# TUI-NICR/EMSANet

Measured on AMD Instinct MI355X. Metric: images/sec (640x480 RGB-D, bs=32/GPU) fwd+bwd, higher is better.
Workload: dtype f32; 1 GPU; BASELINE.json configs[1]: full EMSANet RGB-D (resnet34-NBt1D x2, SE-add fusion, PPM, semantic+instance+orientation+scene heads), 640x480, bs=32/GPU, f32, train mode (BN batch stats, Dropout2d), step = fwd + bwd (fixed output cotangents) + grad all-reduce + SGD-nesterov update at lr 0 (fixed weights) replayed from a hipGraph; global_batch=32, parallelism=dp1, weights=random init (deterministic), mode=train-hipgraph

## Files before the change

### emsanet_amd/_lib.py

```python
import ctypes
import os
from ctypes import POINTER, Structure, c_char_p, c_float, c_int, c_int8, c_int32, c_int64, c_uint32, c_void_p

LIB_PATH = os.environ.get('EMSA_LIB') or os.path.join(
    os.path.dirname(os.path.abspath(__file__)), 'lib', 'libemsanet_hip.so')


class EmsaPackJob(Structure):
    _fields_ = [('src', c_void_p), ('dst0', c_void_p), ('dst1', c_void_p), ('cout', c_int32),
                ('cin', c_int32), ('kh', c_int32), ('kw', c_int32), ('kind', c_int32),
                ('first_block', c_int32), ('cout_total', c_int32), ('cout_off', c_int32),
                ('cin_total', c_int32), ('cin_off', c_int32)]


PACK_GEMM = 0
PACK_WINO = 1
PACK_GEMM_16 = {1: 2, 2: 3}
PACK_COPY = 4
PACK_FRAG_16 = {1: 5, 2: 6}
PACK_WINO2D = 7


class EmsaDropoutJob(Structure):
    _fields_ = [('offset', c_int64), ('c', c_int32), ('layer_id', c_uint32), ('p', c_float),
# ... 14 lines not shown
        ('out_pix_img', c_int32), ('out_pix_row', c_int32), ('out_pix_px', c_int32),
        ('out_pix_off', c_int32),
    ]


class EmsaTargetScale(Structure):
    _fields_ = [('scale', c_int32), ('sigma', c_int32), ('semantic', c_void_p), ('center', c_void_p),
                ('offset', c_void_p), ('foreground', c_void_p), ('orientation', c_void_p),
                ('orientation_foreground', c_void_p)]


class EmsaExportJob(Structure):
    _fields_ = [('src0', c_void_p), ('src1', c_void_p), ('depth', c_void_p), ('lut', c_void_p),
                ('dst', c_void_p), ('divisor', c_int64), ('max_depth', ctypes.c_double),
                ('kind', c_int32), ('src0_dtype', c_int32), ('src1_dtype', c_int32),
                ('depth_dtype', c_int32), ('lut_size', c_int32), ('add', c_int32), ('h', c_int32),
                ('w', c_int32)]


class EmsaNormalScale(Structure):
    _fields_ = [('scale', c_int32), ('reserved', c_int32), ('out', c_void_p)]


_P = c_void_p
_GP = POINTER(EmsaConvGeom)
_TP = POINTER(EmsaTargetScale)

SIGNATURES = {
    'emsa_arch': (c_char_p, []),
    'emsa_version': (c_int, []),
    'emsa_set_batch_invariant': (c_int, [c_int]),
    'emsa_conv_igemm': (c_int, [_GP, _P, _P, _P, _P, _P, _P, _P, _P, c_int32, _P, c_int32, c_int32, _P]),
    'emsa_conv_stats_rows': (c_int, [_GP]),
    'emsa_conv1d_wino_supported': (c_int, [_GP]),
    'emsa_conv1d_wino_stats_rows': (c_int, [_GP]),
    'emsa_conv_relu_bits_words': (c_int64, [c_int64, c_int32]),
    'emsa_conv1d_wino_bnb': (c_int, [_GP, _P, _P, _P, _P, c_int32, _P, c_int32, _P, _P, _P, _P, _P,
                                     c_int32, _P]),
    'emsa_conv_igemm_bnb_t': (c_int, [c_int32, _GP, _P, _P, _P, _P, c_int32, _P, c_int32, _P, _P, _P, _P,
                                      _P, c_int32, _P]),
    'emsa_bn_bwd_apply_rows_t': (c_int, [c_int32, _P, _P, _P, _P, _P, _P, c_int32, c_int32, c_int64,
                                         c_int32, c_int32, _P, _P, _P, _P]),
    'emsa_conv1d_wino': (c_int, [_GP, _P, _P, _P, _P, _P, _P, _P, _P, c_int32, _P, c_int32, c_int32, _P,
                                 _P, _P]),
    'emsa_memset_async': (c_int, [_P, c_int32, c_int64, _P]),
    'emsa_graph_count_nodes': (c_int, [_P, POINTER(c_int32), POINTER(c_int32), POINTER(c_int32)]),
    'emsa_graph_replace_memsets': (c_int, [_P, POINTER(c_int32)]),
    'emsa_dropout2d_mask_batch': (c_int, [_P, _P, c_int32, c_int32, c_int32, c_uint32, _P, _P]),
    'emsa_to_nhwc_t': (c_int, [c_int32, _P, _P, c_int32, c_int32, c_int32, c_int32, c_int64, c_int64,
                               c_int64, c_int64, _P]),
    'emsa_conv1d_wino_set_spec': (c_int, [c_int32]),
    'emsa_wino_set_u_tiled': (c_int, [c_int32]),
    'emsa_conv1d_wino_spec_launches': (c_int, []),
    'emsa_conv1d_wino_resmask_supported': (c_int, [_GP, c_int32]),
    'emsa_conv1d_wino_resmask': (c_int, [_GP, _P, _P, _P, _P, c_int32, _P, _P]),
    'emsa_bn_act_fwd_wbits': (c_int, [_P, _P, _P, _P, _P, _P, c_int32, c_int64, c_int32, c_int32, _P, _P]),
    'emsa_bn_act_fwd_raff': (c_int, [_P] * 8 + [c_int32, c_int64, c_int32, c_int32, _P, c_int32, _P]),
    'emsa_bn_bwd_reduce_wbits': (c_int, [_P, _P, _P, _P, _P, _P, c_int32, c_int64, c_int32, _P, _P]),
    'emsa_bn_bwd_apply_wbits': (c_int, [_P] * 8 + [c_int32, c_int32, c_int64, c_int32, c_int32] + [_P] * 5),
    'emsa_conv1d_wino_inbn': (c_int, [_GP, _P, _P, _P, _P, _P, _P, _P, c_int32, _P, _P]),
    'emsa_conv_wgrad_inbn': (c_int, [_GP, _P, _P, _P, _P, _P, _P, _P, _P]),
    'emsa_conv_wgrad_inbn_t': (c_int, [c_int32, _GP, _P, _P, _P, _P, _P, _P, _P, _P]),
    'emsa_conv_wgrad_multi_inbn_t': (c_int, [c_int32, c_int32, _GP, POINTER(c_void_p), POINTER(c_void_p),
                                             POINTER(c_void_p), POINTER(c_void_p), _P,
                                             POINTER(c_void_p), POINTER(c_void_p), _P]),
    'emsa_conv1d_rs_inbn_t': (c_int, [c_int32, _GP, _P, _P, _P, _P, _P, _P, _P, c_int32, _P]),
    'emsa_bn_bwd_reduce_aff_t': (c_int, [c_int32, _P, _P, _P, _P, _P, _P, c_int32, c_int64, c_int32, _P, _P]),
    'emsa_bn_bwd_apply_aff_t': (c_int, [c_int32, _P, _P, _P, _P, _P, _P, _P, _P, c_int32, c_int32, c_int64,
                                        c_int32, _P, _P, _P, _P]),
    'emsa_conv_wgrad_multi_ws_bytes': (c_int64, [c_int32, c_int32, _GP]),
    'emsa_conv_wgrad_multi_t': (c_int, [c_int32, c_int32, _GP, POINTER(c_void_p), POINTER(c_void_p),
                                        POINTER(c_void_p), POINTER(c_void_p), _P, _P]),
    'emsa_pack_wino': (c_int, [_P, _P, _P, c_int32, c_int32, c_int32, _P]),
    'emsa_pack_batch': (c_int, [_P, c_int32, c_int32, _P]),
    'emsa_conv_wino2d_supported': (c_int, [_GP]),
    'emsa_conv_wino2d_stats_rows': (c_int, [_GP]),
    'emsa_conv_wino2d': (c_int, [_GP, _P, _P, _P, _P, _P, _P, _P, _P, c_int32, _P, c_int32, c_int32, _P]),
    'emsa_conv_wgrad_wino2d_supported': (c_int, [c_int32, _GP]),
    'emsa_conv_wgrad_wino2d_ws_bytes': (c_int64, [c_int32, _GP]),
    'emsa_conv_wgrad_wino2d_split_steps': (c_int, [c_int32, _GP]),
    'emsa_conv_wgrad_wino2d': (c_int, [c_int32, _GP, _P, _P, _P, _P, _P, c_int32, _P]),
    'emsa_pack_wino2d': (c_int, [_P, _P, _P, c_int32, c_int32, _P]),
    'emsa_pack_wino2d_packed': (c_int, [_P, _P, c_int32, c_int32, c_int32, _P]),
    'emsa_pack_wino_packed': (c_int, [_P, _P, c_int32, c_int32, c_int32, c_int32, _P]),
    'emsa_conv_wgrad_ws_bytes': (c_int64, [_GP]),
    'emsa_conv_wgrad': (c_int, [_GP, _P, _P, _P, _P, _P, _P]),
    'emsa_pack_weight_fwd': (c_int, [_P, _P] + [c_int32] * 8 + [_P]),
    'emsa_pack_weight_dgrad': (c_int, [_P, _P] + [c_int32] * 8 + [_P]),
    'emsa_unpack_wgrad': (c_int, [_P, _P] + [c_int32] * 8 + [_P]),
    'emsa_pack_weight_pair': (c_int, [_P, _P, _P] + [c_int32] * 4 + [_P]),
    'emsa_stem_pack_input': (c_int, [_P, _P, c_int32, c_int32, c_int32, c_int32, _P]),
    'emsa_stem_pack_weight': (c_int, [_P, _P, c_int32, c_int32, _P]),
    'emsa_stem_pack_input_rows_t': (c_int, [c_int32, _P, _P, c_int32, c_int32, c_int32, _P]),
    'emsa_stem_pack_weight_rows_t': (c_int, [c_int32, _P, _P, c_int32, _P]),
    'emsa_stem_unpack_wgrad_rows': (c_int, [_P, _P, c_int32, _P]),
    'emsa_stem_unpack_wgrad': (c_int, [_P, _P, c_int32, c_int32, _P]),
    'emsa_bn_finalize': (c_int, [_P, c_int32, c_int32, c_int64, _P, _P, c_float, c_float,
                                 _P, _P, _P, _P, _P, _P, _P, _P]),
    'emsa_bn_finalize_ws_bytes': (c_int, [c_int32]),
    'emsa_bn_fold': (c_int, [_P, _P, _P, _P, c_float, c_int32, _P, _P, _P, _P]),
    'emsa_relu_mask_words': (c_int64, [c_int64]),
    'emsa_bn_act_fwd': (c_int, [_P, _P, _P, _P, _P, _P, c_int32, c_int64, c_int32, c_int32, _P,
                                _P]),
    'emsa_bn_bwd_reduce': (c_int, [_P, _P, _P, _P, _P, _P, _P, c_int32, c_int64, c_int32, c_int32,
                                   _P, _P]),
    'emsa_bn_bwd_rows': (c_int, [c_int64, c_int32]),
# ... 215 lines not shown
```

### emsanet_amd/csrc/conv_wino.hip

```cpp
#include <atomic>
#include <cstdlib>
#include <type_traits>

#include "common.h"
#include "prof.h"

namespace {

constexpr int kWK = 16;
constexpr int kWLD = kWK;
constexpr int kPairs = 32;

typedef unsigned int u32x4w __attribute__((ext_vector_type(4)));
typedef __bf16 wbf16x8 __attribute__((ext_vector_type(8)));
constexpr uint32_t kOOBw = 0x80000000u;
__device__ __forceinline__ __amdgpu_buffer_rsrc_t wrsrc(const void* p, uint32_t bytes) {
  return __builtin_amdgcn_make_buffer_rsrc(const_cast<void*>(p), 0, (int)bytes, 0x00020000);
}
__device__ __forceinline__ float4 wbuf_ld4(__amdgpu_buffer_rsrc_t r, uint32_t off) {
  return __builtin_bit_cast(float4, __builtin_amdgcn_raw_buffer_load_b128(r, (int)off, 0, 0));
}
__device__ __forceinline__ float4 wbuf_ld4s(__amdgpu_buffer_rsrc_t r, uint32_t voff, uint32_t soff) {
  return __builtin_bit_cast(float4,
                            __builtin_amdgcn_raw_buffer_load_b128(r, (int)voff, (int)soff, 0));
}
typedef float wf32x2 __attribute__((ext_vector_type(2)));
typedef unsigned int wu32x2 __attribute__((ext_vector_type(2)));

struct WinoArgs {
  const float* in;
  const float* u;
  float* out;
  const float* bias;
  float* stats;
  const float* scale;
  const float* shift;
  const float* residual;
  const float* mask_src;
  const uint64_t* mask_bits;
  int mask_res;
  uint64_t* relu_bits;
  const float* bnb_mean;
  const float* bnb_invstd;
  float* bnb_out;
  int bnb_rows_alloc;
  const float* in_scale;
  const float* in_shift;
  int ld_out, ld_res, ld_mask, act;
  int L, PL, A, MP;
  int k_ch, n_ch;
  int R, c_in, ksteps_c;
  int u_tiled;
  int in_simg, in_sa, in_sb;
  int px_simg, px_sa, px_sb;
  int tiles_m, tiles_n, ksteps;
  uint32_t in_bytes, u_bytes;
  uint32_t mul_pl, sh_pl, mul_a, sh_a;
};

__device__ __forceinline__ int wswz(int row, int c4) {
  return row * kWLD + (c4 ^ (((row >> 2) & 3) << 2));
}

__device__ __forceinline__ uint32_t wdiv(uint32_t n, uint32_t mul, uint32_t sh) {
  return (__umulhi(n, mul) + n) >> sh;
}

#ifndef EMSA_WINO_ST_AUX
#define EMSA_WINO_ST_AUX 0
#endif
#ifndef EMSA_WINO_PRIO
#define EMSA_WINO_PRIO 2
#endif
enum : int {
  kOBias = 1, kORelu = 2, kORBits = 4, kOStats = 8, kOMBits = 16, kORes = 32, kOMRes = 64
};
template <int kWN, bool BF16 = false, bool BNB = false, bool INBN = false, int OPT = -1>
__global__ __launch_bounds__(256, kWN == 64 ? (BNB ? 4 : 5) : 6) void conv1d_wino_kernel(const WinoArgs p) {
  constexpr bool SPEC = OPT >= 0;
  static_assert(!SPEC || (kWN == 64 && !BF16), "specialised epilogues: fp32, 64-channel tiles");
  const bool f_bias = SPEC ? (OPT & kOBias) != 0 : p.bias != nullptr;
  const bool f_relu = SPEC ? (OPT & kORelu) != 0 : p.act == EMSA_ACT_RELU;
  const bool f_rbits = SPEC ? (OPT & kORBits) != 0 : p.relu_bits != nullptr;
  const bool f_stats = SPEC ? (OPT & kOStats) != 0 : p.stats != nullptr;
  const bool f_mbits = SPEC ? (OPT & kOMBits) != 0 : p.mask_bits != nullptr;
  const bool f_res = SPEC ? (OPT & kORes) != 0 : p.residual != nullptr;
  const bool f_mres = SPEC ? (OPT & kOMRes) != 0 : p.mask_res != 0;
  const bool f_scale = SPEC ? BNB : p.scale != nullptr;
  const bool f_msrc = SPEC ? BNB : p.mask_src != nullptr;
  constexpr int NT = kWN / 32;
  constexpr int NC4 = kWN / 4;
  constexpr int RG = 256 / NC4;
  constexpr int PXI = 64 / RG;
  constexpr int BLD = 4 * kWN * 4 / 256;
  extern __shared__ __attribute__((aligned(16))) float smem[];
  float* const As = smem;
  float* const Bs = smem + 4 * kPairs * kWLD;
  float* const Ts = Bs + 4 * kWN * kWLD;

  const int tid = threadIdx.x, lane = tid & 63, wave = __builtin_amdgcn_readfirstlane(tid >> 6);
  const int l31 = lane & 31, lh = lane >> 5;
  const int wg = emsa_xcd_remap(blockIdx.x, gridDim.x);
  const int nt = wg % p.tiles_n, mt = wg / p.tiles_n;
  const int q0 = mt * kPairs, n0 = nt * kWN;
  const __amdgpu_buffer_rsrc_t rs_in = wrsrc(p.in, p.in_bytes);
  const __amdgpu_buffer_rsrc_t rs_u = wrsrc(p.u, p.u_bytes);

  const int c4 = (tid & 3) * 4;
  uint32_t a_base[2], a_voff[2], b_voff[BLD];
  int a_line[2];
  auto setup_a = [&](int mtile) {
#pragma unroll
    for (int j = 0; j < 2; ++j) {
      const int rowid = (tid >> 2) + 64 * j;
      const int rr = rowid >> 5, pr = rowid & 31;
      const int q = mtile * kPairs + pr;
      uint32_t off = kOOBw;
      int al = 0;
      if (q < p.MP) {
        const int line = (int)wdiv((uint32_t)q, p.mul_pl, p.sh_pl);
        const int pp = q - line * p.PL;
        const int img = (int)wdiv((uint32_t)line, p.mul_a, p.sh_a);
        const int a = line - img * p.A;
        const int b = 2 * pp - 1 + rr;
        if (b >= 0 && b < p.L)
          off = (uint32_t)(img * p.in_simg + a * p.in_sa + b * p.in_sb + c4) * 4u;
        al = a;
      }
      a_base[j] = off;
      a_line[j] = al;
    }
  };
  if constexpr (SPEC) {
    const int rr0 = tid >> 7, q = q0 + ((tid >> 2) & 31);
    a_voff[0] = a_voff[1] = kOOBw;
    if (q < p.MP) {
      const int line = (int)wdiv((uint32_t)q, p.mul_pl, p.sh_pl);
      const int pp = q - line * p.PL;
      const int img = (int)wdiv((uint32_t)line, p.mul_a, p.sh_a);
      const int a = line - img * p.A;
      const int base = img * p.in_simg + a * p.in_sa + c4;
#pragma unroll
      for (int j = 0; j < 2; ++j) {
        const int b = 2 * pp - 1 + rr0 + 2 * j;
        if (b >= 0 && b < p.L) a_voff[j] = (uint32_t)(base + b * p.in_sb) * 4u;
      }
// ... 117 lines not shown
      for (int u = 0; u < NT; ++u) {
        const float4 w0 = emsa_ld4(b + u * 32 * kWLD + c0), w1 = emsa_ld4(b + u * 32 * kWLD + c1);
        wbf16x8 vb;
        vb[0] = (__bf16)w0.x; vb[1] = (__bf16)w0.y; vb[2] = (__bf16)w0.z; vb[3] = (__bf16)w0.w;
        vb[4] = (__bf16)w1.x; vb[5] = (__bf16)w1.y; vb[6] = (__bf16)w1.z; vb[7] = (__bf16)w1.w;
        acc[u] = __builtin_amdgcn_mfma_f32_32x32x16_bf16(va, vb, acc[u], 0, 0, 0);
      }
    } else {
#pragma unroll
    for (int t = 0; t < kWK / 8; ++t) {
      const int co = ((lh + 2 * t) << 2) ^ sw;
      const float4 x0 = emsa_ld4(a0 + co), x1 = emsa_ld4(a1 + co);
      const wf32x2 sg2 = {sg, sg};
      const wf32x2 vlo = __builtin_elementwise_fma(wf32x2{x1.x, x1.y}, sg2, wf32x2{x0.x, x0.y});
      const wf32x2 vhi = __builtin_elementwise_fma(wf32x2{x1.z, x1.w}, sg2, wf32x2{x0.z, x0.w});
      const float4 v = make_float4(vlo.x, vlo.y, vhi.x, vhi.y);
      float4 fb[NT];
#pragma unroll
      for (int u = 0; u < NT; ++u) fb[u] = emsa_ld4(b + u * 32 * kWLD + co);
#pragma unroll
      for (int u = 0; u < NT; ++u) {
        if (first && t == 0) {
          const f32x16 zero = {0.f, 0.f, 0.f, 0.f, 0.f, 0.f, 0.f, 0.f,
                               0.f, 0.f, 0.f, 0.f, 0.f, 0.f, 0.f, 0.f};
          acc[u] = __builtin_amdgcn_mfma_f32_32x32x2f32(v.x, fb[u].x, zero, 0, 0, 0);
        } else {
          acc[u] = __builtin_amdgcn_mfma_f32_32x32x2f32(v.x, fb[u].x, acc[u], 0, 0, 0);
        }
      }
#pragma unroll
      for (int u = 0; u < NT; ++u)
        acc[u] = __builtin_amdgcn_mfma_f32_32x32x2f32(v.y, fb[u].y, acc[u], 0, 0, 0);
#pragma unroll
      for (int u = 0; u < NT; ++u)
        acc[u] = __builtin_amdgcn_mfma_f32_32x32x2f32(v.z, fb[u].z, acc[u], 0, 0, 0);
#pragma unroll
      for (int u = 0; u < NT; ++u)
        acc[u] = __builtin_amdgcn_mfma_f32_32x32x2f32(v.w, fb[u].w, acc[u], 0, 0, 0);
    }
    }
#if EMSA_WINO_PRIO != 0
    __builtin_amdgcn_s_setprio(0);
#endif
    __syncthreads();
    if (has_next) store_lds(s + 1);
    __syncthreads();
  };
  if constexpr (SPEC) {
    kstep(0, std::true_type{});
    for (int s = 1; s < p.ksteps; ++s) kstep(s, std::false_type{});
  } else {
    for (int s = 0; s < p.ksteps; ++s) kstep(s, std::false_type{});
  }

  constexpr int SLD = kWN + 4;
  constexpr int HP = kPairs / 2;
  constexpr uint32_t kNoPix = 0xFFFFFFFFu;
  float* const stage = smem;
  const int col4 = tid % NC4, n = n0 + col4 * 4;
  const int rgi = tid / NC4;
  const bool nok = n < p.n_ch;
  uint32_t lane_pix = kNoPix;
  {
    const int q = q0 + (lane >> 1);
    if (q < p.MP) {
      const int line = (int)wdiv((uint32_t)q, p.mul_pl, p.sh_pl);
      const int pp = q - line * p.PL;
      const int img = (int)wdiv((uint32_t)line, p.mul_a, p.sh_a);
      const int a = line - img * p.A;
      const int b = 2 * pp + (lane & 1);
      if (b < p.L) lane_pix = (uint32_t)(img * p.px_simg + a * p.px_sa + b * p.px_sb);
    }
  }
  wf32x2 ylo[PXI], yhi[PXI];
  uint32_t opix[PXI];
  bool ok[PXI];
  const float4 bv = (nok && f_bias) ? emsa_ld4(p.bias + n) : emsa_zero4();
  const wf32x2 blo = {bv.x, bv.y}, bhi = {bv.z, bv.w};
  const float sgo = (rgi & 1) ? -1.f : 1.f;
  const wf32x2 sg2o = {sgo, sgo};
  const int m03row = (rgi & 1) ? 3 : 0;
#pragma unroll
  for (int k = 0; k < PXI; ++k) {
    const uint32_t o = (uint32_t)__builtin_amdgcn_ds_bpermute((rgi + RG * k) * 4, (int)lane_pix);
    ok[k] = nok && o != kNoPix;
    opix[k] = o;
  }
  const __amdgpu_buffer_rsrc_t rs_out = wrsrc(p.out, kOOBw);
  const __amdgpu_buffer_rsrc_t rs_res = wrsrc(p.residual, kOOBw);
  const __amdgpu_buffer_rsrc_t rs_msk = wrsrc(p.mask_src, kOOBw);
  const __amdgpu_buffer_rsrc_t rs_mb = wrsrc(p.mask_bits, kOOBw);
  float4 rres[PXI], rmsk[PXI];
  wu32x2 rbits[PXI];
#pragma unroll
  for (int k = 0; k < PXI; ++k) {
    const bool live = ok[k];
    if (f_res)
      rres[k] = wbuf_ld4(rs_res, live ? (opix[k] * (uint32_t)p.ld_res + (uint32_t)n) * 4u : kOOBw);
    if (f_msrc)
      rmsk[k] = wbuf_ld4(rs_msk, live ? (opix[k] * (uint32_t)p.ld_mask + (uint32_t)n) * 4u : kOOBw);
    if constexpr (kWN == 64) {
      if (f_mbits)
        rbits[k] = __builtin_bit_cast(
            wu32x2, __builtin_amdgcn_raw_buffer_load_b64(
                        rs_mb, (int)(live ? (opix[k] * (uint32_t)p.tiles_n + (uint32_t)nt) * 8u
                                          : kOOBw), 0, 0));
// ... 445 lines not shown
  if (!(aw || ah || sq)) return 0;
  if (g->mul_h != 1 || g->mul_w != 1 || g->div_h != 1 || g->div_w != 1) return 0;
  if (g->in_h != g->out_h || g->in_w != g->out_w) return 0;
  if ((g->k_ch & 3) || (g->n_ch & 3) || (g->ld_out & 3) || (g->in_px_stride & 3)) return 0;
  if ((long)g->n_img * g->in_img_stride >= (1L << 29)) return 0;
  return 1;
}

extern "C" int64_t emsa_conv_relu_bits_words(int64_t pixels, int32_t n_ch) {
  return pixels * ((n_ch + 63) / 64);
}

extern "C" int emsa_conv1d_wino_stats_rows(const EmsaConvGeom* g) {
  if (!emsa_conv1d_wino_supported(g)) return EMSA_E_SHAPE;
  const bool aw = g->kw == 3;
  const int L = aw ? g->out_w : g->out_h, A = aw ? g->out_h : g->out_w;
  const long mp = (long)g->n_img * A * ((L + 1) / 2);
  return (int)((mp + kPairs - 1) / kPairs);
}

static int wino_wn() {
  static const int forced_wn = [] {
    const char* e = getenv("EMSA_WINO_WN");
    return e ? atoi(e) : 0;
  }();
  return forced_wn == 32 || forced_wn == 64 ? forced_wn : 64;
}

static std::atomic<int> g_wino_spec{[] {
  const char* e = getenv("EMSA_WINO_SPEC");
  return e && e[0] == '0' ? 0 : 1;
}()};
static std::atomic<int> g_wino_spec_launches{0};
extern "C" int emsa_conv1d_wino_set_spec(int32_t on) {
  return g_wino_spec.exchange(on ? 1 : 0, std::memory_order_relaxed);
}
extern "C" int emsa_conv1d_wino_spec_launches(void) {
  return g_wino_spec_launches.load(std::memory_order_relaxed);
}

constexpr int wino_spec_key(bool bnb, bool inbn, int opt) {
  return opt | (bnb ? 0x100 : 0) | (inbn ? 0x200 : 0);
}
static int wino_spec_opt(const WinoArgs& a, int wn, bool bf16) {
  if (!g_wino_spec.load(std::memory_order_relaxed) || wn != 64 || bf16 || a.R != 1 || (a.c_in % kWK)) return -1;
  const bool bnb = a.bnb_out != nullptr;
  if (!bnb && (a.scale || a.mask_src)) return -1;
  if (a.act != EMSA_ACT_NONE && a.act != EMSA_ACT_RELU) return -1;
  const int opt = (a.bias ? kOBias : 0) | (a.act == EMSA_ACT_RELU ? kORelu : 0) |
                  (a.relu_bits ? kORBits : 0) | (a.stats ? kOStats : 0) |
                  (a.mask_bits ? kOMBits : 0) | (a.residual ? kORes : 0) |
                  (a.mask_res ? kOMRes : 0);
  return wino_spec_key(bnb, a.in_scale != nullptr, opt);
}

static int conv1d_wino_impl(const EmsaConvGeom* g, const float* in, const float* u, float* out,
                            const float* bias, float* stats, const float* scale,
                            const float* shift, const float* residual, int32_t ld_res,
                            const float* mask_src, int32_t ld_mask, int32_t act,
                            const uint64_t* mask_bits, uint64_t* relu_bits,
                            const float* bnb_mean, const float* bnb_invstd, float* bnb_out,
                            int32_t bnb_rows_alloc, const float* in_scale, const float* in_shift,
                            void* stream, bool mask_res = false) {
  if (!emsa_conv1d_wino_supported(g)) return EMSA_E_SHAPE;
  if ((in_scale == nullptr) != (in_shift == nullptr)) return EMSA_E_ARG;
  if (!in || !u || !out) return EMSA_E_ARG;
  if ((scale == nullptr) != (shift == nullptr)) return EMSA_E_ARG;
  auto al16 = [](const void* q) { return (((uintptr_t)q) & 15) == 0; };
  if (!al16(out) || !al16(bias) || !al16(scale) || !al16(shift) ||
      (residual && (!al16(residual) || (ld_res & 3))) ||
      (mask_src && (!al16(mask_src) || (ld_mask & 3))))
    return EMSA_E_SHAPE;
  WinoArgs a;
  a.in = in; a.u = u; a.out = out; a.bias = bias; a.stats = stats; a.scale = scale;
  a.shift = shift; a.residual = residual; a.mask_src = mask_src;
  a.mask_bits = mask_bits; a.relu_bits = relu_bits;
  a.mask_res = mask_res ? 1 : 0;
  a.bnb_mean = bnb_mean; a.bnb_invstd = bnb_invstd; a.bnb_out = bnb_out;
  a.bnb_rows_alloc = bnb_rows_alloc;
  a.in_scale = in_scale; a.in_shift = in_shift;
  a.ld_out = g->ld_out; a.ld_res = ld_res; a.ld_mask = ld_mask; a.act = act;
  const bool aw = g->kw == 3;
  const int H = g->out_h, W = g->out_w;
  a.L = aw ? W : H;
  a.A = aw ? H : W;
  a.PL = (a.L + 1) / 2;
  a.MP = g->n_img * a.A * a.PL;
  a.R = g->kh == 3 && g->kw == 3 ? 3 : 1;
  a.c_in = g->k_ch;
  a.k_ch = a.R * g->k_ch; a.n_ch = g->n_ch;
  a.u_tiled = wino_utile_on() && wino_u_tiled(a.R, g->n_ch, g->k_ch) ? 1 : 0;
  a.in_simg = (int)g->in_img_stride;
  a.in_sa = aw ? (int)g->in_row_stride : g->in_px_stride;
  a.in_sb = aw ? g->in_px_stride : (int)g->in_row_stride;
  a.px_simg = H * W;
  a.px_sa = aw ? W : 1;
  a.px_sb = aw ? 1 : W;
  const int wn = wino_wn();
  if ((mask_bits || relu_bits) && wn != 64) return EMSA_E_SHAPE;
  if (mask_bits && mask_src) return EMSA_E_ARG;
  if (mask_res && (!mask_bits || !residual || bnb_out || relu_bits || in_scale)) return EMSA_E_ARG;
  a.tiles_m = (a.MP + kPairs - 1) / kPairs;
  a.tiles_n = (g->n_ch + wn - 1) / wn;
  if (bnb_out) {
    if (!mask_src || !scale || !bnb_mean || !bnb_invstd || mask_bits || relu_bits || stats ||
        act != EMSA_ACT_NONE || !al16(bnb_mean) || bnb_rows_alloc < a.tiles_m)
      return EMSA_E_ARG;
  }
  {
    const long px = (long)g->n_img * H * W, lim = 1L << 29;
    if (px * g->ld_out >= lim || (residual && px * ld_res >= lim) ||
        (mask_src && px * ld_mask >= lim) || px * a.tiles_n * 2 >= lim)
      return EMSA_E_SHAPE;
  }
  a.ksteps_c = (g->k_ch + kWK - 1) / kWK;
  a.ksteps = a.R * a.ksteps_c;
  a.in_bytes = (uint32_t)((size_t)g->n_img * g->in_img_stride * sizeof(float));
  a.u_bytes = (uint32_t)((size_t)4 * g->n_ch * a.k_ch * sizeof(float));
  magic((uint32_t)a.PL, a.mul_pl, a.sh_pl);
  magic((uint32_t)a.A, a.mul_a, a.sh_a);
  if (in_scale && (a.R != 1 || bnb_out || wn != 64)) return EMSA_E_SHAPE;
  const size_t lds_main = (size_t)(4 * kPairs + 4 * wn) * kWLD * sizeof(float) +
                          (in_scale ? (size_t)2 * a.ksteps_c * kWK * sizeof(float) : 0);
  const size_t lds_epi = (size_t)4 * (kPairs / 2) * (wn + 4) * sizeof(float);
  const size_t lds = lds_main > lds_epi ? lds_main : lds_epi;
  const double flops = 2.0 * g->n_img * H * W * (double)g->k_ch * g->n_ch * 3.0 * a.R;
  const int ps = emsa_prof_begin(a.R == 3 ? kProfClassWino3x3 : kProfClassWino, flops,
                                 (hipStream_t)stream);
  static const bool bf16 = [] {
    const char* e = getenv("EMSA_BF16_MFMA");
    return e && e[0] == '1';
  }();
  const dim3 grid(a.tiles_m * a.tiles_n);
#define EMSA_WINO_SPEC_CASE(BNB_, INBN_, OPT_)                                                     \
  case wino_spec_key(BNB_, INBN_, OPT_):                                                           \
    hipLaunchKernelGGL((conv1d_wino_kernel<64, false, BNB_, INBN_, OPT_>), grid, dim3(256), lds,   \
                       (hipStream_t)stream, a);                                                    \
    break;
  bool launched = true;
  switch (wino_spec_opt(a, wn, bf16)) {
    EMSA_WINO_SPEC_CASE(false, false, kOBias | kORelu | kORBits)
    EMSA_WINO_SPEC_CASE(false, true, kOBias | kORelu | kORBits)
    EMSA_WINO_SPEC_CASE(false, false, kOBias | kOStats)
    EMSA_WINO_SPEC_CASE(false, false, kOMBits)
    EMSA_WINO_SPEC_CASE(false, false, kORes | kOMBits | kOMRes)
    EMSA_WINO_SPEC_CASE(false, false, 0)
    EMSA_WINO_SPEC_CASE(true, false, 0)
    EMSA_WINO_SPEC_CASE(true, false, kORes)
    default: launched = false;
  }
#undef EMSA_WINO_SPEC_CASE
  if (launched) {
    g_wino_spec_launches.fetch_add(1, std::memory_order_relaxed);
  } else if (in_scale) {
    hipLaunchKernelGGL((conv1d_wino_kernel<64, false, false, true>),
                       dim3(a.tiles_m * a.tiles_n), dim3(256), lds, (hipStream_t)stream, a);
  } else if (bnb_out) {
    if (wn != 64) return EMSA_E_SHAPE;
    hipLaunchKernelGGL((conv1d_wino_kernel<64, false, true>), dim3(a.tiles_m * a.tiles_n),
                       dim3(256), lds, (hipStream_t)stream, a);
  } else if (wn == 64 && bf16)
    hipLaunchKernelGGL((conv1d_wino_kernel<64, true>), dim3(a.tiles_m * a.tiles_n), dim3(256), lds,
                       (hipStream_t)stream, a);
  else if (wn == 64)
    hipLaunchKernelGGL((conv1d_wino_kernel<64, false>), dim3(a.tiles_m * a.tiles_n), dim3(256),
                       lds, (hipStream_t)stream, a);
  else
    hipLaunchKernelGGL((conv1d_wino_kernel<32, false>), dim3(a.tiles_m * a.tiles_n), dim3(256),
                       lds, (hipStream_t)stream, a);
  emsa_prof_end(ps, (hipStream_t)stream);
  return emsa_launch_status();
}

extern "C" int emsa_conv1d_wino(const EmsaConvGeom* g, const float* in, const float* u, float* out,
                                const float* bias, float* stats, const float* scale,
                                const float* shift, const float* residual, int32_t ld_res,
                                const float* mask_src, int32_t ld_mask, int32_t act,
                                const uint64_t* mask_bits, uint64_t* relu_bits, void* stream) {
  return conv1d_wino_impl(g, in, u, out, bias, stats, scale, shift, residual, ld_res, mask_src,
                          ld_mask, act, mask_bits, relu_bits, nullptr, nullptr, nullptr, 0, nullptr,
                          nullptr, stream);
}

extern "C" int emsa_conv1d_wino_resmask_supported(const EmsaConvGeom* g, int32_t ld_res) {
  if (!emsa_conv1d_wino_supported(g) || wino_wn() != 64) return 0;
  if ((g->n_ch & 63) || ld_res < g->n_ch || (ld_res & 3)) return 0;
  const long px = (long)g->n_img * g->out_h * g->out_w, lim = 1L << 29;
  if (px * g->ld_out >= lim || px * ld_res >= lim || px * (g->n_ch / 64) * 2 >= lim) return 0;
  return 1;
}
extern "C" int emsa_conv1d_wino_resmask(const EmsaConvGeom* g, const float* dy, const float* u,
                                        float* out, const float* residual, int32_t ld_res,
                                        const uint64_t* res_bits, void* stream) {
// ... 29 lines not shown
```

### include/emsanet_hip.h

```cpp
#ifndef EMSANET_HIP_H
#define EMSANET_HIP_H

#include <stdint.h>

#ifdef __cplusplus
extern "C" {
#endif

#define EMSA_OK 0
#define EMSA_E_SHAPE (-1)
#define EMSA_E_ARG (-2)
#define EMSA_E_LAUNCH (-3)

#define EMSA_ACT_NONE 0
#define EMSA_ACT_RELU 1

#define EMSA_DT_F32 0
#define EMSA_DT_BF16 1
#define EMSA_DT_F16 2

const char* emsa_arch(void);
int emsa_version(void);
int emsa_set_batch_invariant(int on);

typedef struct EmsaConvGeom {
  int32_t n_img;
  int32_t in_h, in_w;
  int32_t out_h, out_w;
  int32_t k_ch;
  int32_t n_ch;
  int32_t kh, kw;
  int32_t mul_h, off_h, step_h, div_h;
  int32_t mul_w, off_w, step_w, div_w;
  int64_t in_img_stride, in_row_stride;
  int32_t in_px_stride;
  int32_t ld_out;
  int32_t out_pix_img, out_pix_row, out_pix_px, out_pix_off;
} EmsaConvGeom;

int emsa_conv_igemm(const EmsaConvGeom* g, const float* in, const float* w, float* out,
                    const float* bias, float* stats, const float* scale, const float* shift,
                    const float* residual, int32_t ld_res, const float* mask_src,
                    int32_t ld_mask, int32_t act, void* stream);
int emsa_conv_stats_rows(const EmsaConvGeom* g);

int64_t emsa_conv_wgrad_ws_bytes(const EmsaConvGeom* g);
int emsa_conv_wgrad(const EmsaConvGeom* g, const float* in, const float* dout, float* dw,
                    float* dbias, float* ws, void* stream);

int emsa_conv1d_wino_supported(const EmsaConvGeom* g);
int emsa_conv1d_wino_stats_rows(const EmsaConvGeom* g);
int64_t emsa_conv_relu_bits_words(int64_t pixels, int32_t n_ch);
int emsa_conv1d_wino(const EmsaConvGeom* g, const float* in, const float* u, float* out,
                     const float* bias, float* stats, const float* scale, const float* shift,
                     const float* residual, int32_t ld_res, const float* mask_src,
                     int32_t ld_mask, int32_t act, const uint64_t* mask_bits,
                     uint64_t* relu_bits, void* stream);
int emsa_conv1d_wino_bnb(const EmsaConvGeom* g, const float* dy, const float* u, float* out,
                         const float* residual, int32_t ld_res, const float* t, int32_t ld_t,
                         const float* bn_scale, const float* bn_shift, const float* bn_mean,
                         const float* bn_invstd, float* partial, int32_t rows_alloc, void* stream);
int emsa_conv1d_wino_set_spec(int32_t on);
int emsa_conv1d_wino_spec_launches(void);
int emsa_wino_set_u_tiled(int32_t on);
int emsa_conv1d_wino_resmask_supported(const EmsaConvGeom* g, int32_t ld_res);
int emsa_conv1d_wino_resmask(const EmsaConvGeom* g, const float* dy, const float* u, float* out,
                             const float* residual, int32_t ld_res, const uint64_t* res_bits,
                             void* stream);
int emsa_conv1d_wino_inbn(const EmsaConvGeom* g, const float* in, const float* u, float* out,
                          const float* bias, float* stats, const float* in_scale,
                          const float* in_shift, int32_t act, uint64_t* relu_bits, void* stream);
int emsa_conv_wgrad_inbn(const EmsaConvGeom* g, const float* in, const float* dout, float* dw,
                         float* dbias, float* ws, const float* in_scale, const float* in_shift,
                         void* stream);
int emsa_pack_wino(const float* w_oihw, float* u, float* u_dgrad, int32_t cout, int32_t cin,
                   int32_t rows, void* stream);
int emsa_pack_wino_packed(const float* w_packed, float* u, int32_t n_ch, int32_t k_ch,
                          int32_t rows, int32_t flip, void* stream);
int emsa_conv_wino2d_supported(const EmsaConvGeom* g);
int emsa_conv_wino2d_stats_rows(const EmsaConvGeom* g);
int emsa_conv_wino2d(const EmsaConvGeom* g, const float* in, const float* u2, float* out,
                     const float* bias, float* stats, const float* scale, const float* shift,
                     const float* residual, int32_t ld_res, const float* mask_src,
                     int32_t ld_mask, int32_t act, void* stream);
int emsa_conv_wgrad_wino2d_supported(int32_t dtype, const EmsaConvGeom* g);
int64_t emsa_conv_wgrad_wino2d_ws_bytes(int32_t dtype, const EmsaConvGeom* g);
int emsa_conv_wgrad_wino2d_split_steps(int32_t dtype, const EmsaConvGeom* g);
int emsa_conv_wgrad_wino2d(int32_t dtype, const EmsaConvGeom* g, const void* in, const void* dout,
                           float* dw, float* dbias, float* ws, int32_t packed, void* stream);
int emsa_pack_wino2d(const float* w_oihw, float* u, float* u_dgrad, int32_t cout, int32_t cin,
                     void* stream);
int emsa_pack_wino2d_packed(const float* w_packed, float* u, int32_t n_ch, int32_t k_ch,
                            int32_t flip, void* stream);
typedef struct EmsaPackJob {
  const float* src;
  float* dst0;
  float* dst1;
  int32_t cout, cin, kh, kw;
  int32_t kind;
  int32_t first_block;
  int32_t cout_total, cout_off, cin_total, cin_off;
} EmsaPackJob;
int emsa_pack_batch(const EmsaPackJob* jobs_device, int32_t n_jobs, int32_t total_blocks,
                    void* stream);

int emsa_pack_weight_fwd(const float* w_oihw, float* w_packed, int32_t cout, int32_t cin,
                         int32_t kh, int32_t kw, int32_t cout_total, int32_t cout_off,
                         int32_t cin_total, int32_t cin_off,
                         void* stream);
int emsa_pack_weight_dgrad(const float* w_oihw, float* w_packed, int32_t cout, int32_t cin,
                           int32_t kh, int32_t kw, int32_t cout_total, int32_t cout_off,
                           int32_t cin_total, int32_t cin_off,
                           void* stream);
int emsa_pack_weight_pair(const float* w_oihw, float* w_packed_fwd, float* w_packed_dgrad,
                          int32_t cout, int32_t cin, int32_t kh, int32_t kw, void* stream);
int emsa_unpack_wgrad(const float* dw_packed, float* dw_oihw, int32_t cout, int32_t cin,
// ... 577 lines not shown
```

Before: 358.2 images/s.

## Add persistent 64-channel Winograd 1D conv kernel with register-resident weights

Adds a persistent-grid kernel for 64-in/64-out 1D Winograd convolutions. It keeps the transformed weights in registers for the whole kernel and loops over pixel tiles, prefetching the next input tile while the MFMA work runs. The shared epilogue is factored into a separate device function. The goal is to stop reloading weights per tile and to hide load latency, at the cost of higher register pressure (3 blocks/CU) and extra LDS. By default it is enabled only when the tile count is large enough to give many rounds per resident block.

```diff
diff --git a/emsanet_amd/_lib.py b/emsanet_amd/_lib.py
--- a/emsanet_amd/_lib.py
+++ b/emsanet_amd/_lib.py
@@ -90,6 +90,9 @@
     'emsa_conv1d_wino_set_spec': (c_int, [c_int32]),
     'emsa_wino_set_u_tiled': (c_int, [c_int32]),
     'emsa_conv1d_wino_spec_launches': (c_int, []),
+    'emsa_conv1d_wino_set_c64': (c_int, [c_int32]),
+    'emsa_conv1d_wino_set_c64_grid': (c_int, [c_int32]),
+    'emsa_conv1d_wino_c64_launches': (c_int, []),
     'emsa_conv1d_wino_resmask_supported': (c_int, [_GP, c_int32]),
     'emsa_conv1d_wino_resmask': (c_int, [_GP, _P, _P, _P, _P, c_int32, _P, _P]),
     'emsa_bn_act_fwd_wbits': (c_int, [_P, _P, _P, _P, _P, _P, c_int32, c_int64, c_int32, c_int32, _P, _P]),
diff --git a/emsanet_amd/csrc/conv_wino.hip b/emsanet_amd/csrc/conv_wino.hip
--- a/emsanet_amd/csrc/conv_wino.hip
+++ b/emsanet_amd/csrc/conv_wino.hip
@@ -75,23 +75,14 @@
 enum : int {
   kOBias = 1, kORelu = 2, kORBits = 4, kOStats = 8, kOMBits = 16, kORes = 32, kOMRes = 64
 };
+template <int kWN, bool BNB, int OPT>
+__device__ __forceinline__ void wino_epilogue(const WinoArgs& p, f32x16 (&acc)[kWN / 32],
+                                              float* smem, int mt, int nt, int tid);
 template <int kWN, bool BF16 = false, bool BNB = false, bool INBN = false, int OPT = -1>
 __global__ __launch_bounds__(256, kWN == 64 ? (BNB ? 4 : 5) : 6) void conv1d_wino_kernel(const WinoArgs p) {
   constexpr bool SPEC = OPT >= 0;
   static_assert(!SPEC || (kWN == 64 && !BF16), "specialised epilogues: fp32, 64-channel tiles");
-  const bool f_bias = SPEC ? (OPT & kOBias) != 0 : p.bias != nullptr;
-  const bool f_relu = SPEC ? (OPT & kORelu) != 0 : p.act == EMSA_ACT_RELU;
-  const bool f_rbits = SPEC ? (OPT & kORBits) != 0 : p.relu_bits != nullptr;
-  const bool f_stats = SPEC ? (OPT & kOStats) != 0 : p.stats != nullptr;
-  const bool f_mbits = SPEC ? (OPT & kOMBits) != 0 : p.mask_bits != nullptr;
-  const bool f_res = SPEC ? (OPT & kORes) != 0 : p.residual != nullptr;
-  const bool f_mres = SPEC ? (OPT & kOMRes) != 0 : p.mask_res != 0;
-  const bool f_scale = SPEC ? BNB : p.scale != nullptr;
-  const bool f_msrc = SPEC ? BNB : p.mask_src != nullptr;
   constexpr int NT = kWN / 32;
-  constexpr int NC4 = kWN / 4;
-  constexpr int RG = 256 / NC4;
-  constexpr int PXI = 64 / RG;
   constexpr int BLD = 4 * kWN * 4 / 256;
   extern __shared__ __attribute__((aligned(16))) float smem[];
   float* const As = smem;
@@ -315,6 +306,182 @@
   } else {
     for (int s = 0; s < p.ksteps; ++s) kstep(s, std::false_type{});
   }
+  wino_epilogue<kWN, BNB, OPT>(p, acc, smem, mt, nt, tid);
+}
+
+template <bool BNB, bool INBN, int OPT>
+__global__ __launch_bounds__(256, 3) void conv1d_wino_c64_kernel(const WinoArgs p) {
+  constexpr int kImg = 4 * kPairs * kWLD + 16;
+  extern __shared__ __attribute__((aligned(16))) float smem[];
+  float* const As = smem;
+  float* const Ts = smem + 4 * kImg;
+  float* const Es = Ts + 128;
+  const int tid = threadIdx.x, lane = tid & 63, wave = __builtin_amdgcn_readfirstlane(tid >> 6);
+  const int l31 = lane & 31, lh = lane >> 5;
+  const int grid = (int)gridDim.x;
+  int mt = emsa_xcd_remap(blockIdx.x, grid);
+  const __amdgpu_buffer_rsrc_t rs_in = wrsrc(p.in, p.in_bytes);
+  const __amdgpu_buffer_rsrc_t rs_u = wrsrc(p.u, p.u_bytes);
+
+  const int pr = tid >> 3, c8 = (tid & 7) * 4;
+  const int ls = (tid & 7) >> 2, lc4 = (tid & 3) * 4;
+  uint32_t a_voff[4];
+  float4 ra[4][2];
+  auto load_tile = [&](int mtile) {
+    const int q = mtile * kPairs + pr;
+#pragma unroll
+    for (int r = 0; r < 4; ++r) a_voff[r] = kOOBw;
+    if (q < p.MP) {
+      uint32_t mul_pl = p.mul_pl, mul_a = p.mul_a;
+      asm volatile("" : "+s"(mul_pl), "+s"(mul_a));
+      const int line = (int)wdiv((uint32_t)q, mul_pl, p.sh_pl);
+      const int pp = q - line * p.PL;
+      const int img = (int)wdiv((uint32_t)line, mul_a, p.sh_a);
+      const int a = line - img * p.A;
+      const int base = img * p.in_simg + a * p.in_sa + c8;
+#pragma unroll
+      for (int r = 0; r < 4; ++r) {
+        const int b = 2 * pp - 1 + r;
+        if (b >= 0 && b < p.L) a_voff[r] = (uint32_t)(base + b * p.in_sb) * 4u;
+      }
+    }
+#pragma unroll
+    for (int r = 0; r < 4; ++r)
+#pragma unroll
+      for (int h = 0; h < 2; ++h) ra[r][h] = wbuf_ld4s(rs_in, a_voff[r], (uint32_t)h * 128u);
+  };
+  auto store_lds = [&]() {
+#pragma unroll
+    for (int h = 0; h < 2; ++h) {
+      float4 sc, sh;
+      if constexpr (INBN) {
+        sc = emsa_ld4(Ts + c8 + 32 * h);
+        sh = emsa_ld4(Ts + 64 + c8 + 32 * h);
+      }
+#pragma unroll
+      for (int r = 0; r < 4; ++r) {
+        float4 v = ra[r][h];
+        if constexpr (INBN) {
+          const float cap = __uint_as_float(0x7F800000u & ~(uint32_t)((int32_t)a_voff[r] >> 31));
+          const wf32x2 lo = __builtin_elementwise_fma(wf32x2{v.x, v.y}, wf32x2{sc.x, sc.y},
+                                                      wf32x2{sh.x, sh.y});
+          const wf32x2 hi = __builtin_elementwise_fma(wf32x2{v.z, v.w}, wf32x2{sc.z, sc.w},
+                                                      wf32x2{sh.z, sh.w});
+          v = make_float4(__builtin_amdgcn_fmed3f(lo.x, 0.f, cap),
+                          __builtin_amdgcn_fmed3f(lo.y, 0.f, cap),
+                          __builtin_amdgcn_fmed3f(hi.x, 0.f, cap),
+                          __builtin_amdgcn_fmed3f(hi.y, 0.f, cap));
+        }
+        emsa_st4(As + (ls + 2 * h) * kImg + wswz(r * kPairs + pr, lc4), v);
+      }
+    }
+  };
+
+  float4 ur[4][2][2];
+  {
+    const uint32_t uv = (uint32_t)(l31 * kWLD + 4 * lh) * 4u;
+#pragma unroll
+    for (int s = 0; s < 4; ++s)
+#pragma unroll
+      for (int t = 0; t < 2; ++t)
+#pragma unroll
+        for (int u = 0; u < 2; ++u)
+          ur[s][t][u] = wbuf_ld4s(rs_u, uv, (uint32_t)(s * 16384 + wave * 4096 +
+                                                       (u * 32 * kWLD + 8 * t) * 4));
+  }
+  load_tile(mt);
+  if constexpr (INBN) {
+    if (tid < 64) {
+      Ts[tid] = p.in_scale[tid];
+      Ts[64 + tid] = p.in_shift[tid];
+    }
+    __syncthreads();
+  }
+
+  const int ra_ = wave == 0 ? 0 : wave == 2 ? 2 : 1;
+  const int rb_ = wave == 2 ? 1 : wave == 3 ? 3 : 2;
+  const float sg = wave == 1 ? 1.f : -1.f;
+  const wf32x2 sg2 = {sg, sg};
+  const int sw = ((l31 >> 2) & 3) << 2;
+  const float* const a0 = As + (ra_ * kPairs + l31) * kWLD;
+  const float* const a1 = As + (rb_ * kPairs + l31) * kWLD;
+
+  store_lds();
+  for (;;) {
+    __syncthreads();
+    const int mt_next = mt + grid;
+#if EMSA_WINO_PRIO == 2
+    __builtin_amdgcn_s_setprio(3);
+#endif
+    load_tile(mt_next);
+#if EMSA_WINO_PRIO != 0
+    __builtin_amdgcn_s_setprio(1);
+#endif
+    f32x16 acc[2];
+#pragma unroll
+    for (int s = 0; s < 4; ++s) {
+#pragma unroll
+      for (int t = 0; t < 2; ++t) {
+        const int co = ((lh + 2 * t) << 2) ^ sw;
+        const float4 x0 = emsa_ld4(a0 + s * kImg + co), x1 = emsa_ld4(a1 + s * kImg + co);
+        const wf32x2 vlo = __builtin_elementwise_fma(wf32x2{x1.x, x1.y}, sg2, wf32x2{x0.x, x0.y});
+        const wf32x2 vhi = __builtin_elementwise_fma(wf32x2{x1.z, x1.w}, sg2, wf32x2{x0.z, x0.w});
+        const float4 v = make_float4(vlo.x, vlo.y, vhi.x, vhi.y);
+#pragma unroll
+        for (int u = 0; u < 2; ++u) {
+          if (s == 0 && t == 0) {
+            const f32x16 zero = {0.f, 0.f, 0.f, 0.f, 0.f, 0.f, 0.f, 0.f,
+                                 0.f, 0.f, 0.f, 0.f, 0.f, 0.f, 0.f, 0.f};
+            acc[u] = __builtin_amdgcn_mfma_f32_32x32x2f32(v.x, ur[s][t][u].x, zero, 0, 0, 0);
+          } else {
+            acc[u] = __builtin_amdgcn_mfma_f32_32x32x2f32(v.x, ur[s][t][u].x, acc[u], 0, 0, 0);
+          }
+        }
+#pragma unroll
+        for (int u = 0; u < 2; ++u)
+          acc[u] = __builtin_amdgcn_mfma_f32_32x32x2f32(v.y, ur[s][t][u].y, acc[u], 0, 0, 0);
+#pragma unroll
+        for (int u = 0; u < 2; ++u)
+          acc[u] = __builtin_amdgcn_mfma_f32_32x32x2f32(v.z, ur[s][t][u].z, acc[u], 0, 0, 0);
+#pragma unroll
+        for (int u = 0; u < 2; ++u)
+          acc[u] = __builtin_amdgcn_mfma_f32_32x32x2f32(v.w, ur[s][t][u].w, acc[u], 0, 0, 0);
+      }
+    }
+#if EMSA_WINO_PRIO != 0
+    __builtin_amdgcn_s_setprio(0);
+#endif
+    __syncthreads();
+    store_lds();
+    int etid = tid;
+    asm volatile("" : "+v"(etid));
+    wino_epilogue<64, BNB, OPT>(p, acc, Es, mt, 0, etid);
+    if (mt_next >= p.tiles_m) break;
+    mt = mt_next;
+  }
+}
+
+template <int kWN, bool BNB, int OPT>
+__device__ __forceinline__ void wino_epilogue(const WinoArgs& p, f32x16 (&acc)[kWN / 32],
+                                              float* const smem, const int mt, const int nt,
+                                              const int tid) {
+  constexpr bool SPEC = OPT >= 0;
+  const bool f_bias = SPEC ? (OPT & kOBias) != 0 : p.bias != nullptr;
+  const bool f_relu = SPEC ? (OPT & kORelu) != 0 : p.act == EMSA_ACT_RELU;
+  const bool f_rbits = SPEC ? (OPT & kORBits) != 0 : p.relu_bits != nullptr;
+  const bool f_stats = SPEC ? (OPT & kOStats) != 0 : p.stats != nullptr;
+  const bool f_mbits = SPEC ? (OPT & kOMBits) != 0 : p.mask_bits != nullptr;
+  const bool f_res = SPEC ? (OPT & kORes) != 0 : p.residual != nullptr;
+  const bool f_mres = SPEC ? (OPT & kOMRes) != 0 : p.mask_res != 0;
+  const bool f_scale = SPEC ? BNB : p.scale != nullptr;
+  const bool f_msrc = SPEC ? BNB : p.mask_src != nullptr;
+  constexpr int NT = kWN / 32;
+  constexpr int NC4 = kWN / 4;
+  constexpr int RG = 256 / NC4;
+  constexpr int PXI = 64 / RG;
+  const int lane = tid & 63, wave = __builtin_amdgcn_readfirstlane(tid >> 6);
+  const int l31 = lane & 31, lh = lane >> 5;
+  const int q0 = mt * kPairs, n0 = nt * kWN;
 
   constexpr int SLD = kWN + 4;
   constexpr int HP = kPairs / 2;
@@ -866,6 +1033,49 @@
                   (a.mask_bits ? kOMBits : 0) | (a.residual ? kORes : 0) |
                   (a.mask_res ? kOMRes : 0);
   return wino_spec_key(bnb, a.in_scale != nullptr, opt);
+}
+
+static std::atomic<int> g_wino_c64{[] {
+  const char* e = getenv("EMSA_WINO_C64");
+  return e && e[0] >= '0' && e[0] <= '2' ? e[0] - '0' : 1;
+}()};
+static std::atomic<int> g_wino_c64_grid{0};
+static std::atomic<int> g_wino_c64_launches{0};
+extern "C" int emsa_conv1d_wino_set_c64(int32_t mode) {
+  return g_wino_c64.exchange(mode < 0 ? 0 : mode > 2 ? 2 : mode, std::memory_order_relaxed);
+}
+extern "C" int emsa_conv1d_wino_set_c64_grid(int32_t n) {
+  return g_wino_c64_grid.exchange(n > 0 ? n : 0, std::memory_order_relaxed);
+}
+extern "C" int emsa_conv1d_wino_c64_launches(void) {
+  return g_wino_c64_launches.load(std::memory_order_relaxed);
+}
+constexpr int kC64Resident = 3;
+constexpr int kC64MinRounds = 8;
+static int wino_c64_grid(const WinoArgs& a, int key) {
+  const int mode = g_wino_c64.load(std::memory_order_relaxed);
+  if (!mode || key < 0 || a.R != 1 || a.c_in != 64 || a.n_ch != 64 || !a.u_tiled) return 0;
+  switch (key) {
+    case wino_spec_key(false, false, kOBias | kORelu | kORBits):
+    case wino_spec_key(false, true, kOBias | kORelu | kORBits):
+    case wino_spec_key(false, false, kOBias | kOStats):
+    case wino_spec_key(false, false, kOMBits):
+    case wino_spec_key(false, false, kORes | kOMBits | kOMRes):
+    case wino_spec_key(true, false, 0): break;
+    default: return 0;
+  }
+  static const int cus = [] {
+    int dev = 0, n = 0;
+    if (hipGetDevice(&dev) != hipSuccess ||
+        hipDeviceGetAttribute(&n, hipDeviceAttributeMultiprocessorCount, dev) != hipSuccess || n <= 0)
+      n = 256;
+    return n;
+  }();
+  const int full = cus * kC64Resident;
+  if (mode == 1 && a.tiles_m < kC64MinRounds * full) return 0;
+  const int cap = g_wino_c64_grid.load(std::memory_order_relaxed);
+  const int grid = cap > 0 && cap < full ? cap : full;
+  return a.tiles_m < grid ? a.tiles_m : grid;
 }
 
 static int conv1d_wino_impl(const EmsaConvGeom* g, const float* in, const float* u, float* out,
@@ -952,7 +1162,26 @@
                        (hipStream_t)stream, a);                                                    \
     break;
   bool launched = true;
-  switch (wino_spec_opt(a, wn, bf16)) {
+  const int key = wino_spec_opt(a, wn, bf16);
+  const int c64_grid = wino_c64_grid(a, key);
+  if (c64_grid) {
+    const size_t lds64 = (size_t)(4 * (4 * kPairs * kWLD + 16) + 128) * sizeof(float) + lds_epi;
+#define EMSA_WINO_C64_CASE(BNB_, INBN_, OPT_)                                                      \
+  case wino_spec_key(BNB_, INBN_, OPT_):                                                           \
+    hipLaunchKernelGGL((conv1d_wino_c64_kernel<BNB_, INBN_, OPT_>), dim3(c64_grid), dim3(256),     \
+                       lds64, (hipStream_t)stream, a);                                             \
+    break;
+    switch (key) {
+      EMSA_WINO_C64_CASE(false, false, kOBias | kORelu | kORBits)
+      EMSA_WINO_C64_CASE(false, true, kOBias | kORelu | kORBits)
+      EMSA_WINO_C64_CASE(false, false, kOBias | kOStats)
+      EMSA_WINO_C64_CASE(false, false, kOMBits)
+      EMSA_WINO_C64_CASE(false, false, kORes | kOMBits | kOMRes)
+      EMSA_WINO_C64_CASE(true, false, 0)
+    }
+#undef EMSA_WINO_C64_CASE
+    g_wino_c64_launches.fetch_add(1, std::memory_order_relaxed);
+  } else switch (key) {
     EMSA_WINO_SPEC_CASE(false, false, kOBias | kORelu | kORBits)
     EMSA_WINO_SPEC_CASE(false, true, kOBias | kORelu | kORBits)
     EMSA_WINO_SPEC_CASE(false, false, kOBias | kOStats)
diff --git a/include/emsanet_hip.h b/include/emsanet_hip.h
--- a/include/emsanet_hip.h
+++ b/include/emsanet_hip.h
@@ -62,6 +62,9 @@
                          const float* bn_invstd, float* partial, int32_t rows_alloc, void* stream);
 int emsa_conv1d_wino_set_spec(int32_t on);
 int emsa_conv1d_wino_spec_launches(void);
+int emsa_conv1d_wino_set_c64(int32_t mode);
+int emsa_conv1d_wino_set_c64_grid(int32_t n);
+int emsa_conv1d_wino_c64_launches(void);
 int emsa_wino_set_u_tiled(int32_t on);
 int emsa_conv1d_wino_resmask_supported(const EmsaConvGeom* g, int32_t ld_res);
 int emsa_conv1d_wino_resmask(const EmsaConvGeom* g, const float* dy, const float* u, float* out,
```

Result: no change. 359.7 images/s, median of 6 (+0.4%).
